# YuHang-max/3DSAD-main

Hardware: AMD Instinct MI355X
Metric: scenes/sec (16384-pt KITTI-shaped) through SA+cluster path (higher is better)
Workload: dtype f32

## Files before the change

3dsad-main_amd/csrc/mlp_layer.hip:

```cpp
#include "common.h"
#include <map>
#include <mutex>
#include <utility>

namespace {

#include "reg_common.h"

constexpr int LWAVES = 4;
constexpr int SLOTS = 16;

using sad::LayerJob;
using sad::LayerMulti;

#ifndef SAD_LAYER_KC
#define SAD_LAYER_KC 2
#endif
constexpr int KC = SAD_LAYER_KC;
constexpr int STAGE_F4 = KC * 8 * 64;

__device__ __forceinline__ int job_rows(const LayerJob &jb) { return jb.rowtab ? jb.rowtab[0] : jb.rows; }

struct RowInfo {
    int q, grp;
    bool live, whole;
    unsigned xoff;
    float4 rel;
};
template <bool GATHER>
__device__ __forceinline__ RowInfo row_info(const LayerJob &jb, int rt, int lane, bool need_gid) {
    RowInfo r;
    const int j = lane & 31, h = lane >> 5;
    const int total = job_rows(jb);
    r.q = rt * 32 + j;
    r.live = r.q < total;
    if (!r.live) r.q = total - 1;
    int src = r.q, gv = 0;
    if (GATHER || need_gid) gv = jb.row_gid[r.q];
    if (GATHER) src = jb.row_src[r.q];
    r.grp = gv & (WHOLE_BIT - 1);
    r.whole = (gv & WHOLE_BIT) != 0;
    r.xoff = (unsigned)src * (unsigned)jb.ldx * 4u;
    r.rel = make_float4(0.f, 0.f, 0.f, 0.f);
    if (GATHER && h == 0) {
        const float *pq = jb.xyz + (long long)src * 3;
        const float *pc = jb.new_xyz + (long long)r.grp * 3;
        r.rel = make_float4(pq[0] - pc[0], pq[1] - pc[1], pq[2] - pc[2], 0.f);
    }
    return r;
}

struct Chunk { float4 a0, a1, a2, a3, b0, b1, b2, b3; };
static_assert(KC == 4 || KC == 2, "Chunk holds up to four activation fragments");

template <bool GATHER>
__device__ __forceinline__ Chunk load_chunk_of(const LayerJob &jb, const unsigned xoff, const int ob, const int c, const int wave, const int lane) {
    const int h = lane >> 5;
    const int KG = jb.kg;
    const char *xb = reinterpret_cast<const char *>(jb.x);
    const float4 *wf = reinterpret_cast<const float4 *>(jb.packed + jb.off + jb.np) + (size_t)(ob * 4) * KG * 64;
    const unsigned ulane = (unsigned)lane;
    float4 ga[4], gb[KC];
#pragma unroll
    for (int i = 0; i < KC; ++i) {
        const int f = wave * KC + i;
        const int gk = c * KC + (f >> 2);
        ga[i] = (wf + ((size_t)(f & 3) * KG + (gk < KG ? gk : KG - 1)) * 64)[ulane];
    }
#pragma unroll
    for (int u = 0; u < KC; ++u) {
        int g = c * KC + u;
        g = g < KG ? g : KG - 1;
        if constexpr (GATHER) {
            const int ch = 2 * g - 1 + h;
            const int cc = ch < 0 ? 0 : (ch < jb.cpr ? ch : jb.cpr - 1);
            gb[u] = *reinterpret_cast<const float4 *>(xb + (size_t)(xoff + 16u * (unsigned)cc));
        } else {
#if defined(SAD_LAYER_WHATIF) && SAD_LAYER_WHATIF >= 3
            gb[u] = make_float4(0.25f, 0.5f, 0.75f, 1.f);
#elif defined(SAD_LAYER_WHATIF) && SAD_LAYER_WHATIF == 2
            gb[u] = *reinterpret_cast<const float4 *>((xb + (size_t)g * 32) + (size_t)(16u * (unsigned)h));
#else
            gb[u] = *reinterpret_cast<const float4 *>((xb + (size_t)g * 32) + (size_t)(xoff + 16u * (unsigned)h));
#endif
        }
    }
    return Chunk{ga[0], ga[1], ga[KC > 2 ? 2 : 0], ga[KC > 2 ? 3 : 0], gb[0], gb[1], gb[KC > 2 ? 2 : 0], gb[KC > 2 ? 3 : 0]};
}

struct Prefetched {
    Chunk ck;
    float4 rel;
    unsigned xoff;
    int valid;
    int next;
};
struct NextItem {
    int ji;
    int rb, ob;
};
struct NextSource {
    int dyn;
    int pulled;
    int stat;
    int own;
};
constexpr int META_ITEM = 0, META_I0 = 1, META_N = 2;

template <bool GATHER, bool LAST>
__device__ __forceinline__ Prefetched gemm_item(const LayerMulti &lm, const LayerJob &jb, const int rb, const int ob, float4 *lds,
                                                const Prefetched pin, const NextSource ns) {
    Prefetched pre;
    pre.valid = 0;
    pre.next = 0x7FFFFFFF;
    int *meta = reinterpret_cast<int *>(lds + 2 * STAGE_F4);
    auto publish_next = [&]() {
        if (ns.dyn && threadIdx.x == 0) meta[META_ITEM] = ns.pulled * 8 + ns.own;
    };
    const int tid = threadIdx.x, lane = tid & 63, wave = __builtin_amdgcn_readfirstlane(tid >> 6);
    const int h = lane >> 5;
    const int wy = wave >> 1, wx = wave & 1;
    const int KG = jb.kg;
    const int NC = (KG + KC - 1) / KC;
    unsigned fr_xoff;
    float4 fr_rel;
    if (pin.valid) {
        fr_xoff = pin.xoff;
        fr_rel = pin.rel;
    } else {
        const RowInfo fr = row_info<GATHER>(jb, rb * 4 + wave, lane, false);
        fr_xoff = fr.xoff;
        fr_rel = fr.rel;
    }
    auto load_chunk = [&](int c) -> Chunk { return load_chunk_of<GATHER>(jb, fr_xoff, ob, c, wave, lane); };
    auto store_chunk = [&](const Chunk ck, int c, float4 *st) {
        const float4 ga[4] = {ck.a0, ck.a1, ck.a2, ck.a3}, gb[4] = {ck.b0, ck.b1, ck.b2, ck.b3};
#pragma unroll
        for (int i = 0; i < KC; ++i) {
            const int f = wave * KC + i;
            st[((f >> 2) * 8 + (f & 3)) * 64 + lane] = ga[i];
        }
#pragma unroll
        for (int u = 0; u < KC; ++u) {
            const int g = c * KC + u;
            float4 v = gb[u];
            if constexpr (GATHER) {
                const int ch = 2 * g - 1 + h;
                const bool ok = ch >= 0 && ch < jb.cpr;
                v.x = ok ? v.x : 0.f; v.y = ok ? v.y : 0.f; v.z = ok ? v.z : 0.f; v.w = ok ? v.w : 0.f;
                const bool first = g == 0 && h == 0;
                v.x = first ? fr_rel.x : v.x; v.y = first ? fr_rel.y : v.y; v.z = first ? fr_rel.z : v.z; v.w = first ? fr_rel.w : v.w;
            }
            if (g >= KG) v = make_float4(0.f, 0.f, 0.f, 0.f);
            float ops[4];
            to_operands(v.x, v.y, v.z, v.w, ops);
            st[(u * 8 + 4 + wave) * 64 + lane] = make_float4(ops[0], ops[1], ops[2], ops[3]);
        }
    };
    f32x16 acc[2][2];
    {
        const float *bias = jb.packed + jb.off + (ob * 4 + 2 * wx) * 32;
#pragma unroll
        for (int oc = 0; oc < 2; ++oc)
#pragma unroll
            for (int a = 0; a < 4; ++a) {
                const float4 bv = *reinterpret_cast<const float4 *>(bias + oc * 32 + 8 * a + 4 * h);
#pragma unroll
                for (int rt = 0; rt < 2; ++rt) {
                    acc[rt][oc][4 * a + 0] = bv.x; acc[rt][oc][4 * a + 1] = bv.y; acc[rt][oc][4 * a + 2] = bv.z; acc[rt][oc][4 * a + 3] = bv.w;
                }
            }
    }
    __syncthreads();
    Chunk nxt;
    if (pin.valid) nxt = pin.ck;
    else nxt = load_chunk(0);
    store_chunk(nxt, 0, lds);
    if (NC == 1) publish_next();
    __syncthreads();
#if defined(SAD_LAYER_WHATIF) && SAD_LAYER_WHATIF == 4
    float4 wnx[2], xnx[2];
    wnx[0] = wnx[1] = xnx[0] = xnx[1] = make_float4(0.f, 0.f, 0.f, 0.f);
#endif
#pragma unroll 1
    for (int c = 0; c < NC; ++c) {
        float4 *cur = lds + (c & 1) * STAGE_F4;
        if (c + 1 < NC) {
            nxt = load_chunk(c + 1);
        } else {
          const int nitem = __builtin_amdgcn_readfirstlane(ns.dyn ? meta[META_ITEM] : ns.stat);
          const int mi0 = __builtin_amdgcn_readfirstlane(meta[META_I0]);
          pre.next = nitem;
          if (nitem < __builtin_amdgcn_readfirstlane(meta[META_N])) {
            const int nji = nitem < mi0 ? 0 : 1;
            const int nit = nitem - (nji ? mi0 : 0);
            const int nnog = nji ? lm.j[1].nog : lm.j[0].nog;
            NextItem nx;
            nx.ji = nji;
            nx.rb = nit / nnog;
            nx.ob = nit % nnog;
#define SAD_FETCH_NEXT(NJ)                                                                         \
    do {                                                                                           \
        if ((NJ).gather) {                                                                         \
            const RowInfo nf = row_info<true>((NJ), nx.rb * 4 + wave, lane, false);                \
            pre.xoff = nf.xoff;                                                                    \
            pre.rel = nf.rel;                                                                      \
            pre.ck = load_chunk_of<true>((NJ), nf.xoff, nx.ob, 0, wave, lane);                     \
        } else {                                                                                   \
            const RowInfo nf = row_info<false>((NJ), nx.rb * 4 + wave, lane, false);               \
            pre.xoff = nf.xoff;                                                                    \
            pre.rel = nf.rel;                                                                      \
            pre.ck = load_chunk_of<false>((NJ), nf.xoff, nx.ob, 0, wave, lane);                    \
        }                                                                                          \
    } while (0)
            if (nx.ji == 0) SAD_FETCH_NEXT(lm.j[0]);
            else SAD_FETCH_NEXT(lm.j[1]);
#undef SAD_FETCH_NEXT
            pre.valid = 1;
          }
        }
        float4 wa[2][2], xa[2][2];
#if defined(SAD_LAYER_WHATIF) && SAD_LAYER_WHATIF == 4
        if (c == 0) {
#endif
#pragma unroll
        for (int i = 0; i < 2; ++i) {
            wa[0][i] = cur[(0 * 8 + 2 * wx + i) * 64 + lane];
            xa[0][i] = cur[(0 * 8 + 4 + 2 * wy + i) * 64 + lane];
        }
#if defined(SAD_LAYER_WHATIF) && SAD_LAYER_WHATIF == 4
        } else {
#pragma unroll
            for (int i = 0; i < 2; ++i) { wa[0][i] = wnx[i]; xa[0][i] = xnx[i]; }
        }
#endif
#pragma unroll
        for (int u = 0; u < KC; ++u) {
            if (u + 1 < KC) {
#pragma unroll
                for (int i = 0; i < 2; ++i) {
                    wa[(u + 1) & 1][i] = cur[((u + 1) * 8 + 2 * wx + i) * 64 + lane];
                    xa[(u + 1) & 1][i] = cur[((u + 1) * 8 + 4 + 2 * wy + i) * 64 + lane];
                }
            }
            __builtin_amdgcn_sched_barrier(0);
#pragma unroll
            for (int rt = 0; rt < 2; ++rt) {
                const float ops[4] = {xa[u & 1][rt].x, xa[u & 1][rt].y, xa[u & 1][rt].z, xa[u & 1][rt].w};
#pragma unroll
                for (int oc = 0; oc < 2; ++oc) acc[rt][oc] = mma4(acc[rt][oc], wa[u & 1][oc], ops);
            }
            __builtin_amdgcn_sched_barrier(0);
        }
        if (c + 1 < NC) store_chunk(nxt, c + 1, lds + ((c + 1) & 1) * STAGE_F4);
        if (c + 2 == NC) publish_next();
#if defined(SAD_LAYER_WHATIF) && SAD_LAYER_WHATIF == 4
        {
            const float4 *nx = lds + ((c + 1) & 1) * STAGE_F4;
#pragma unroll
            for (int i = 0; i < 2; ++i) {
                wnx[i] = nx[(0 * 8 + 2 * wx + i) * 64 + lane];
                xnx[i] = nx[(0 * 8 + 4 + 2 * wy + i) * 64 + lane];
            }
        }
#endif
        __syncthreads();
    }
    if (jb.relu) {
#pragma unroll
        for (int rt = 0; rt < 2; ++rt)
#pragma unroll
            for (int oc = 0; oc < 2; ++oc)
#pragma unroll
                for (int g = 0; g < 16; ++g) acc[rt][oc][g] = acc[rt][oc][g] > 0.f ? acc[rt][oc][g] : 0.f;
    }
#pragma unroll
    for (int rt = 0; rt < 2; ++rt) {
        const RowInfo ri = row_info<false>(jb, rb * 4 + 2 * wy + rt, lane, LAST);
        const int j = lane & 31;
        if constexpr (!LAST) {
#if defined(SAD_LAYER_WHATIF) && SAD_LAYER_WHATIF >= 1
            if (ri.live && ri.q == 0x7FFFFFF0) {
#else
            if (ri.live) {
#endif
                float *yrow = jb.y + (long long)ri.q * jb.ldy + (ob * 4 + 2 * wx) * 32 + 4 * h;
#pragma unroll
                for (int oc = 0; oc < 2; ++oc)
#pragma unroll
                    for (int a = 0; a < 4; ++a)
                        *reinterpret_cast<float4 *>(yrow + oc * 32 + 8 * a) =
                            make_float4(acc[rt][oc][4 * a], acc[rt][oc][4 * a + 1], acc[rt][oc][4 * a + 2], acc[rt][oc][4 * a + 3]);
            }
        } else {
            float *stage = reinterpret_cast<float *>(lds) + wave * (SLOTS * 64);
            const int key = ri.live ? ri.grp + 1 : 0;
            const PoolMasks pm = pool_masks(key);
            const int nkey = __shfl_down(key, 1, 64), pkey = __shfl_up(key, 1, 64);
            const bool tail = ri.live && (j == 31 || nkey != key);
            const bool head = ri.live && (j == 0 || pkey != key);
            const unsigned heads = (unsigned)__ballot(head), tails = (unsigned)__ballot(tail);
            const int ngroups = __builtin_popcount(heads);
            const int slot = __builtin_popcount(heads & (0xFFFFFFFFu >> (31 - j))) - 1;
            const bool staged = ngroups <= SLOTS;
            const int ch0 = (ob * 4 + 2 * wx) * 32;
#pragma unroll
            for (int oc = 0; oc < 2; ++oc) {
                const f32x16 t = seg_max16(acc[rt][oc], pm);
                if (!tail) continue;
                if (staged) {
                    float *d = stage + slot * 64 + oc * 32 + 4 * h;
#pragma unroll
                    for (int a = 0; a < 4; ++a) *reinterpret_cast<float4 *>(d + 8 * a) = make_float4(t[4 * a], t[4 * a + 1], t[4 * a + 2], t[4 * a + 3]);
                } else {
                    float *o = jb.out + (long long)ri.grp * jb.ld_out + jb.col_off + ch0 + oc * 32 + 4 * h;
#pragma unroll
                    for (int a = 0; a < 4; ++a)
#pragma unroll
                        for (int e = 0; e < 4; ++e) {
                            if (ch0 + oc * 32 + 8 * a + 4 * h + e >= jb.cout_last) continue;
                            if (ri.whole) o[8 * a + e] = t[4 * a + e];
                            else atomic_max_pos(o + 8 * a + e, t[4 * a + e]);
                        }
                }
            }
            if (staged) {
                unsigned rem = tails;
                for (int s = 0; s < ngroups; ++s) {
                    const int p = __builtin_ctz(rem);
                    rem &= rem - 1;
                    const int g = __builtin_amdgcn_readlane(ri.grp, p);
                    const bool w = __builtin_amdgcn_readlane((int)ri.whole, p) != 0;
                    float *orow = jb.out + (long long)g * jb.ld_out + jb.col_off + ch0;
                    const float *sp = stage + s * 64;
                    if (ch0 + lane < jb.cout_last) {
                        if (w) orow[lane] = sp[lane];
                        else atomic_max_pos(orow + lane, sp[lane]);
                    }
                }
            }
        }
    }
    return pre;
}

__global__ __launch_bounds__(LWAVES * 64) __attribute__((amdgpu_waves_per_eu(2, 2))) void mlp_layer_kernel(const LayerMulti lm) {
    extern __shared__ __attribute__((aligned(16))) float4 lds4[];
    int *meta = reinterpret_cast<int *>(lds4 + 2 * STAGE_F4);
    const int i0 = ((job_rows(lm.j[0]) + 127) / 128) * lm.j[0].nog;
    const int nitems = lm.n > 1 ? i0 + ((job_rows(lm.j[1]) + 127) / 128) * lm.j[1].nog : i0;
    const int dyn = lm.queue != nullptr;
    const sad::ItemQueue Q = sad::itemq_init(lm.queue, dyn ? 8 : 0);
    int item = blockIdx.x;
    if (threadIdx.x == 0) {
        meta[META_I0] = i0;
        meta[META_N] = nitems;
        if (dyn) meta[META_ITEM] = sad::itemq_item(Q, Q.own, sad::itemq_pull(Q));
    }
    __syncthreads();
    if (dyn) item = meta[META_ITEM];
    Prefetched pre;
    pre.valid = 0;
    while (true) {
        if (item >= nitems) {
            if (!dyn) break;
            __syncthreads();
            if (threadIdx.x == 0) meta[META_ITEM] = sad::itemq_steal(Q, nitems);
            __syncthreads();
            item = meta[META_ITEM];
            if (item >= nitems) break;
            pre.valid = 0;
        }
        const int ji = item < i0 ? 0 : 1;
        const int it = item - (ji ? i0 : 0);
        const LayerJob &jb = lm.j[ji];
        const int nog = jb.nog;
        NextSource ns;
        ns.dyn = dyn;
        ns.pulled = 0;
        if (dyn && threadIdx.x == 0) ns.pulled = sad::itemq_pull(Q);
        ns.stat = item + (int)gridDim.x;
        ns.own = Q.own;
        if (jb.gather) {
            if (jb.last) pre = gemm_item<true, true>(lm, jb, it / nog, it % nog, lds4, pre, ns);
            else pre = gemm_item<true, false>(lm, jb, it / nog, it % nog, lds4, pre, ns);
        } else {
            if (jb.last) pre = gemm_item<false, true>(lm, jb, it / nog, it % nog, lds4, pre, ns);
            else pre = gemm_item<false, false>(lm, jb, it / nog, it % nog, lds4, pre, ns);
        }
        item = pre.next;
    }
    if (dyn && threadIdx.x == 0) sad::itemq_done(Q, (int)gridDim.x);
}

}

namespace sad {

int *stream_item_queue(hipStream_t st) {
    static std::mutex mu;
    static std::map<std::pair<int, hipStream_t>, int *> queues;
    hipStreamCaptureStatus cap = hipStreamCaptureStatusNone;
    if (hipStreamIsCapturing(st, &cap) != hipSuccess || cap != hipStreamCaptureStatusNone) {
        (void)hipGetLastError();
        return nullptr;
    }
    int dev = 0;
    if (hipGetDevice(&dev) != hipSuccess) {
        (void)hipGetLastError();
        return nullptr;
    }
    std::lock_guard<std::mutex> lk(mu);
    auto it = queues.find({dev, st});
    if (it != queues.end()) return it->second;
    int *q = nullptr;
    if (hipMalloc(&q, sizeof(int) * ITEMQ_INTS) != hipSuccess) {
        (void)hipGetLastError();
        return nullptr;
    }
    if (hipMemsetAsync(q, 0, sizeof(int) * ITEMQ_INTS, st) != hipSuccess) {
        (void)hipGetLastError();
        (void)hipFree(q);
        return nullptr;
    }
    queues[{dev, st}] = q;
    return q;
}

int launch_layers(const LayerMulti &lm_in, long long max_items, hipStream_t st) {
    LayerMulti lm = lm_in;
    lm.queue = get_option(OPT_MLP_LAYER_QUEUE) == 1 ? stream_item_queue(st) : nullptr;
    static std::atomic<uint64_t> attr_done{0};
    lds_attr_once(attr_done, reinterpret_cast<const void *>(&mlp_layer_kernel), 160 * 1024);
    const size_t lds = sizeof(float4) * ((size_t)2 * STAGE_F4 + 1);
    static std::atomic<int> per_cu{0};
    int pc = per_cu.load(std::memory_order_relaxed);
    if (pc == 0) {
        int nb = 0;
        if (hipOccupancyMaxActiveBlocksPerMultiprocessor(&nb, mlp_layer_kernel, LWAVES * 64, lds) != hipSuccess || nb < 1) {
            (void)hipGetLastError();
            nb = 2;
        }
        pc = nb > 2 ? 2 : nb;
        per_cu.store(pc, std::memory_order_relaxed);
    }
    if (get_option(OPT_MLP_DYN_SLOTS) > 0 && get_option(OPT_MLP_DYN_SLOTS) < pc) pc = get_option(OPT_MLP_DYN_SLOTS);
    const int cus = sad::device_cus();
    long long grid = (long long)cus * pc;
    const long long cap = max_items;
    if (grid > cap) grid = cap < 1 ? 1 : cap;
    hipLaunchKernelGGL(mlp_layer_kernel, dim3((unsigned)grid), dim3(LWAVES * 64), lds, st, lm);
    return check_launch("sad_mlp_chain_f32 (layer-streamed chain)");
}

}
```

3dsad-main_amd/csrc/reg_common.h:

```cpp
#pragma once
#include "prims.h"

constexpr int WHOLE_BIT = 1 << 30;
using sad::RegChain;
using sad::RegMulti;

struct Swapped { float lo, hi; };
__device__ __forceinline__ Swapped swap32(float a, float b) {
    const auto r = __builtin_amdgcn_permlane32_swap(__builtin_bit_cast(unsigned, a), __builtin_bit_cast(unsigned, b), false, false);
    const unsigned r0 = r[0], r1 = r[1];
    return {__builtin_bit_cast(float, r0), __builtin_bit_cast(float, r1)};
}

__device__ __forceinline__ void to_operands(float v0, float v1, float v2, float v3, float *out) {
    const Swapped s01 = swap32(v0, v1);
    const Swapped s23 = swap32(v2, v3);
    out[0] = s01.lo;
    out[1] = s23.lo;
    out[2] = s01.hi;
    out[3] = s23.hi;
}

__device__ __forceinline__ f32x16 mma4(f32x16 acc, const float4 a, const float *b) {
    acc = __builtin_amdgcn_mfma_f32_32x32x2f32(a.x, b[0], acc, 0, 0, 0);
    acc = __builtin_amdgcn_mfma_f32_32x32x2f32(a.y, b[1], acc, 0, 0, 0);
    acc = __builtin_amdgcn_mfma_f32_32x32x2f32(a.z, b[2], acc, 0, 0, 0);
    acc = __builtin_amdgcn_mfma_f32_32x32x2f32(a.w, b[3], acc, 0, 0, 0);
    return acc;
}

__device__ __forceinline__ f32x16 bias_tile(const float *sb, int h) {
    f32x16 t;
#pragma unroll
    for (int a = 0; a < 4; ++a) {
        const float4 bv = *reinterpret_cast<const float4 *>(sb + 8 * a + 4 * h);
        t[4 * a + 0] = bv.x; t[4 * a + 1] = bv.y; t[4 * a + 2] = bv.z; t[4 * a + 3] = bv.w;
    }
    return t;
}

__device__ __forceinline__ f32x16 relu16(f32x16 t) {
#pragma unroll
    for (int g = 0; g < 16; ++g) t[g] = __builtin_amdgcn_fmed3f(t[g], 0.f, __builtin_inff());
    return t;
}

template <int CTRL, int ROWMASK>
__device__ __forceinline__ int dpp_i(int v) {
    return __builtin_amdgcn_update_dpp(0, v, CTRL, ROWMASK, 0xF, true);
}

struct PoolMasks {
    bool m[5];
    bool any[5];
};

__device__ __forceinline__ PoolMasks pool_masks(int key) {
    PoolMasks pm;
    pm.m[0] = dpp_i<0x111, 0xF>(key) == key;
    pm.m[1] = dpp_i<0x112, 0xF>(key) == key;
    pm.m[2] = dpp_i<0x114, 0xF>(key) == key;
    pm.m[3] = dpp_i<0x118, 0xF>(key) == key;
    pm.m[4] = dpp_i<0x142, 0xA>(key) == key;
#pragma unroll
    for (int k = 0; k < 5; ++k) pm.any[k] = __ballot(pm.m[k]) != 0;
    return pm;
}

__device__ __forceinline__ f32x16 seg_max16(f32x16 t, const PoolMasks &pm) {
#ifdef SAD_NOSCAN
    return t;
#endif
    unsigned x[16];
#pragma unroll
    for (int g = 0; g < 16; ++g) {
        const float f = t[g];
        x[g] = __builtin_bit_cast(unsigned, f);
    }
#define SAD_STEP(CTRL, RM, K)                                                   \
    if (pm.any[K]) {                                                            \
        _Pragma("unroll") for (int g = 0; g < 16; ++g) {                        \
            const unsigned u = (unsigned)dpp_i<CTRL, RM>((int)x[g]);            \
            const unsigned r = u > x[g] ? u : x[g];                             \
            x[g] = pm.m[K] ? r : x[g];                                          \
        }                                                                       \
    }
    SAD_STEP(0x111, 0xF, 0)
    SAD_STEP(0x112, 0xF, 1)
    SAD_STEP(0x114, 0xF, 2)
    SAD_STEP(0x118, 0xF, 3)
    SAD_STEP(0x142, 0xA, 4)
#undef SAD_STEP
#pragma unroll
    for (int g = 0; g < 16; ++g) t[g] = __builtin_bit_cast(float, x[g]);
    return t;
}

__device__ __forceinline__ void pool_store(f32x16 t, const PoolMasks &pm, bool tail, bool whole, float *orow, int o, int h,
                                           const RegChain &c) {
#ifdef SAD_REG_NOPOOL
    if (t[0] == 123.f) orow[0] = t[0];
    return;
#endif
    t = seg_max16(t, pm);
#ifdef SAD_REG_NOSTORE
    {
        float s = 0.f;
#pragma unroll
        for (int g = 0; g < 16; ++g) s += t[g];
        if (s == 123.456f) orow[0] = s;
        return;
    }
#endif
#ifdef SAD_REG_NOATOMIC
    whole = true;
#endif
    if (tail) {
#pragma unroll
        for (int a = 0; a < 4; ++a) {
            const int ch = o * 32 + 8 * a + 4 * h;
            if (whole && c.vec_out && ch + 3 < c.cout_last) {
                *reinterpret_cast<float4 *>(orow + ch) = make_float4(t[4 * a], t[4 * a + 1], t[4 * a + 2], t[4 * a + 3]);
            } else {
#pragma unroll
                for (int e = 0; e < 4; ++e) {
                    if (ch + e >= c.cout_last) continue;
                    if (whole) orow[ch + e] = t[4 * a + e];
                    else atomic_max_pos(orow + ch + e, t[4 * a + e]);
                }
            }
        }
    }
}

struct Stage {
    float *lds;
    int slot;
    unsigned tails;
    int ngroups;
};

template <int COUT>
__device__ __forceinline__ void pool_stage(f32x16 t, const PoolMasks &pm, bool tail, const Stage &sg, int o, int h) {
#ifdef SAD_REG_NOPOOL
    if (t[0] == 123.f) sg.lds[0] = t[0];
    return;
#endif
    t = seg_max16(t, pm);
#ifdef SAD_REG_NOSTORE
    {
        float s = 0.f;
#pragma unroll
        for (int g = 0; g < 16; ++g) s += t[g];
        if (s == 123.456f) sg.lds[0] = s;
        return;
    }
#endif
    if (tail) {
        float *d = sg.lds + sg.slot * COUT + o * 32 + 4 * h;
#pragma unroll
        for (int a = 0; a < 4; ++a)
            *reinterpret_cast<float4 *>(d + 8 * a) = make_float4(t[4 * a], t[4 * a + 1], t[4 * a + 2], t[4 * a + 3]);
    }
}

template <int COUT>
__device__ __forceinline__ void stage_flush(const Stage &sg, int grp, bool whole, int lane, const RegChain &c) {
#if defined(SAD_REG_NOPOOL) || defined(SAD_REG_NOSTORE)
    return;
#endif
    unsigned rem = sg.tails;
    for (int s = 0; s < sg.ngroups; ++s) {
        const int p = __builtin_ctz(rem);
        rem &= rem - 1;
        const int g = __builtin_amdgcn_readlane(grp, p);
        const bool w = __builtin_amdgcn_readlane((int)whole, p) != 0;
        float *orow = c.out + (long long)g * c.ld_out + c.col_off;
        const float *src = sg.lds + s * COUT;
        if (w && c.vec_out && COUT == c.cout_last) {
            if (lane * 4 < COUT) *reinterpret_cast<float4 *>(orow + lane * 4) = *reinterpret_cast<const float4 *>(src + lane * 4);
        } else {
#pragma unroll
            for (int k = 0; k < (COUT + 63) / 64; ++k) {
                const int ch = lane + 64 * k;
                if (ch < COUT && ch < c.cout_last) {
                    if (w) orow[ch] = src[ch];
                    else atomic_max_pos(orow + ch, src[ch]);
                }
            }
        }
    }
}
```

Measured before the change: 8527.

## Flush pooled groups in parallel across lanes and tweak relu and segmented max

For small output widths, stage_flush now stores several whole groups at once. It builds a slot-to-group lookup table with ds_permute and gives each lane a float4 of one group, so the old serial loop that wrote one group per iteration is gone. Only the first and last groups, which may be partial, still go through the atomic path. ReLU now uses an integer sign comparison instead of fmed3 or a select. The segmented max splits the DPP max and the mask select into separate passes with sched_barriers, which changes the instruction schedule. The new flush path assumes only the boundary groups can be non-whole, and the barriers may limit how the compiler interleaves instructions.

```diff
diff --git a/3dsad-main_amd/csrc/mlp_layer.hip b/3dsad-main_amd/csrc/mlp_layer.hip
--- a/3dsad-main_amd/csrc/mlp_layer.hip
+++ b/3dsad-main_amd/csrc/mlp_layer.hip
@@ -270,9 +270,7 @@
 #pragma unroll
         for (int rt = 0; rt < 2; ++rt)
 #pragma unroll
-            for (int oc = 0; oc < 2; ++oc)
-#pragma unroll
-                for (int g = 0; g < 16; ++g) acc[rt][oc][g] = acc[rt][oc][g] > 0.f ? acc[rt][oc][g] : 0.f;
+            for (int oc = 0; oc < 2; ++oc) acc[rt][oc] = relu16(acc[rt][oc]);
     }
 #pragma unroll
     for (int rt = 0; rt < 2; ++rt) {
diff --git a/3dsad-main_amd/csrc/reg_common.h b/3dsad-main_amd/csrc/reg_common.h
--- a/3dsad-main_amd/csrc/reg_common.h
+++ b/3dsad-main_amd/csrc/reg_common.h
@@ -41,7 +41,11 @@
 
 __device__ __forceinline__ f32x16 relu16(f32x16 t) {
 #pragma unroll
-    for (int g = 0; g < 16; ++g) t[g] = __builtin_amdgcn_fmed3f(t[g], 0.f, __builtin_inff());
+    for (int g = 0; g < 16; ++g) {
+        const float f = t[g];
+        const int b = __builtin_bit_cast(int, f);
+        t[g] = __builtin_bit_cast(float, b > 0 ? b : 0);
+    }
     return t;
 }
 
@@ -71,7 +75,7 @@
 #ifdef SAD_NOSCAN
     return t;
 #endif
-    unsigned x[16];
+    unsigned x[16], u[16];
 #pragma unroll
     for (int g = 0; g < 16; ++g) {
         const float f = t[g];
@@ -79,11 +83,14 @@
     }
 #define SAD_STEP(CTRL, RM, K)                                                   \
     if (pm.any[K]) {                                                            \
+        __builtin_amdgcn_sched_barrier(0);                                      \
         _Pragma("unroll") for (int g = 0; g < 16; ++g) {                        \
-            const unsigned u = (unsigned)dpp_i<CTRL, RM>((int)x[g]);            \
-            const unsigned r = u > x[g] ? u : x[g];                             \
-            x[g] = pm.m[K] ? r : x[g];                                          \
+            const unsigned d = (unsigned)dpp_i<CTRL, RM>((int)x[g]);            \
+            u[g] = d > x[g] ? d : x[g];                                         \
         }                                                                       \
+        __builtin_amdgcn_sched_barrier(0);                                      \
+        _Pragma("unroll") for (int g = 0; g < 16; ++g) x[g] = pm.m[K] ? u[g] : x[g]; \
+        __builtin_amdgcn_sched_barrier(0);                                      \
     }
     SAD_STEP(0x111, 0xF, 0)
     SAD_STEP(0x112, 0xF, 1)
@@ -169,12 +176,8 @@
 #if defined(SAD_REG_NOPOOL) || defined(SAD_REG_NOSTORE)
     return;
 #endif
-    unsigned rem = sg.tails;
-    for (int s = 0; s < sg.ngroups; ++s) {
-        const int p = __builtin_ctz(rem);
-        rem &= rem - 1;
+    auto one_group = [&](int s, int p, bool w) {
         const int g = __builtin_amdgcn_readlane(grp, p);
-        const bool w = __builtin_amdgcn_readlane((int)whole, p) != 0;
         float *orow = c.out + (long long)g * c.ld_out + c.col_off;
         const float *src = sg.lds + s * COUT;
         if (w && c.vec_out && COUT == c.cout_last) {
@@ -189,5 +192,30 @@
                 }
             }
         }
-    }
-}
+    };
+    constexpr int LPG = COUT / 4;
+    if (COUT <= 64 && c.vec_out && COUT == c.cout_last) {
+        constexpr int G = 64 / LPG;
+        const bool tail_lo = lane < 32 && ((sg.tails >> lane) & 1u) != 0;
+        const int tab = __builtin_amdgcn_ds_permute((tail_lo ? sg.slot : 63) << 2, grp | (whole ? WHOLE_BIT : 0));
+        const int sub = lane / LPG;
+        float *const obase = c.out + c.col_off + (lane % LPG) * 4;
+        const long long ld = c.ld_out;
+        const float4 *src = reinterpret_cast<const float4 *>(sg.lds) + lane;
+        for (int s0 = 0; s0 < sg.ngroups; s0 += G, src += 64) {
+            const int s = s0 + sub;
+            const int gv = __builtin_amdgcn_ds_bpermute(s << 2, tab);
+            if (s < sg.ngroups && (gv & WHOLE_BIT) != 0) *reinterpret_cast<float4 *>(obase + (gv & (WHOLE_BIT - 1)) * ld) = *src;
+        }
+        const int p0 = __builtin_ctz(sg.tails), p1 = 31 - __builtin_clz(sg.tails);
+        if (__builtin_amdgcn_readlane((int)whole, p0) == 0) one_group(0, p0, false);
+        if (sg.ngroups > 1 && __builtin_amdgcn_readlane((int)whole, p1) == 0) one_group(sg.ngroups - 1, p1, false);
+    } else {
+        unsigned rem = sg.tails;
+        for (int s = 0; s < sg.ngroups; ++s) {
+            const int p = __builtin_ctz(rem);
+            rem &= rem - 1;
+            one_group(s, p, __builtin_amdgcn_readlane((int)whole, p) != 0);
+        }
+    }
+}
```

After: 8458. No clear change (-0.8%).
